# casinca/LLM-quest

Measured on AMD Instinct MI355X. Metric: img+tokens/sec fwd+bwd, ViT-B+Qwen3-0.6B VLM, 224px+512tok, higher is better.
Workload: dtype bf16; 1 GPU; BASELINE configs[3]: VLM early fusion, ViT-B/16 (frozen, fwd) + ffn adapter 768->3072->1024 + Qwen3-0.6B, 224x224 image + 512 text tokens (S=709), fwd+loss+bwd, no optimizer step; per_gpu_batch=160, global_batch=160, parallelism=dp1, text_mask=all ones, vision_tower_precision=bf16 MFMA operands, fp32 residual stream

## Files before the change

### llm_quest_amd/csrc/attention.hip

```cpp
#include "attn_common.h"

namespace {

template <int D>
__global__ __launch_bounds__(256, 2) void attn_fwd_kernel(int B, int S, int Hq, int Hkv, const bf16_t* __restrict__ q, int64_t ldq,
                                                          const bf16_t* __restrict__ k, int64_t ldk, const bf16_t* __restrict__ v,
                                                          int64_t ldv, bf16_t* __restrict__ o, int64_t ldo, float* __restrict__ lse,
                                                          const uint8_t* __restrict__ key_mask, int causal, float scale_log2) {
    using C = Cfg<D>;
    const int abl = causal >> 8;
    causal &= 0xff;
    __shared__ __attribute__((aligned(16))) char smem[4 * C::TILE];
    const int lane = threadIdx.x & 63;
    const int wave = __builtin_amdgcn_readfirstlane(threadIdx.x >> 6);
    const int nqb = (S + 127) / 128;
    const int vid = (abl >> 8) & 1 ? (int)blockIdx.x : xcd_chunked((int)blockIdx.x, (int)gridDim.x);
    const int qb = nqb - 1 - (vid % nqb);
    const int bh = vid / nqb;
    const int hq = bh % Hq, b = bh / Hq;
    const int hkv = hq / (Hq / Hkv);
    const int q0 = qb * 128;
    const int qg = q0 + wave * 32 + (lane & 31);
    const bool qvalid = qg < S;

// ... 282 lines not shown

    for (int kt = 0; kt < ntiles; ++kt) {
        [[maybe_unused]] const unsigned long long t_sync = PROF_T();
        wait_vmcnt<0>();
        __syncthreads();
        PROF_ADD(1, t_sync);
        const int nv = S - kt * 64;
        unsigned long long kbits = nv >= 64 ? ~0ull : ((1ull << nv) - 1ull);
        if (mrow) kbits &= __ballot(mk != 0);
        [[maybe_unused]] const unsigned long long t_iss = PROF_T();
        const bool more = kt + 1 < ntiles;
        const bool spread = more && S - (kt + 1) * 64 >= 64 && !(abl & 512);
        if (more && !spread) issue(kt + 1, (kt + 1) & 1);
        const auto nkr = __builtin_amdgcn_make_buffer_rsrc(const_cast<bf16_t*>(kbase + (int64_t)(kt + 1) * 64 * ldk), 0, 0x7fffffff, 0x00020000);
        const auto nvr = __builtin_amdgcn_make_buffer_rsrc(const_cast<bf16_t*>(vbase + (int64_t)(kt + 1) * 64 * ldv), 0, 0x7fffffff, 0x00020000);
        char* const nst = smem + ((kt + 1) & 1) * 2 * C::TILE;
        auto piece = [&](auto i_) {
            constexpr int i = i_.value;
            if constexpr (i < C::PPW) {
                const int row = (wave * C::PPW + i) * C::RPP + prow;
                __builtin_amdgcn_raw_ptr_buffer_load_lds(nkr, LDS_PTR(nst + (wave * C::PPW + i) * 1024), 16, dk_row + (unsigned)(swz_row<D>(pch, row) << 4), (int)(i * C::RPP * ldk * 2), 0, 0);
            } else {
                constexpr int j = i - C::PPW;
                const int row = (wave * C::PPW + j) * C::RPP + prow;
                __builtin_amdgcn_raw_ptr_buffer_load_lds(nvr, LDS_PTR(nst + C::TILE + (wave * C::PPW + j) * 1024), 16, dv_row + (unsigned)(swz_tr<D>(pch, row) << 4), (int)(j * C::RPP * ldv * 2), 0, 0);
            }
        };
        PROF_ADD(2, t_iss);
        if (mrow) mk = mrow[min((kt + 1) * 64 + lane, S - 1)];
        [[maybe_unused]] unsigned long long t_seg = PROF_T();
        if (prof_on) prof_acc[7] += 1;
        const int koff = (kt & 1) * 2 * C::TILE, voff = koff + C::TILE;
        if (causal && !allt && kt * 64 > qw + 31) continue;
        int vkx[C::KS], vv[C::DT];
#pragma unroll
        for (int ks = 0; ks < C::KS; ++ks) vkx[ks] = (lo.row + koff) ^ (ks << 5);
#pragma unroll
        for (int dt = 0; dt < C::DT; ++dt) vv[dt] = lo.col[dt] + voff;
        f32x16 sacc[2];
        static_assert(2 * C::PPW == C::KS, "one next-tile piece behind every second MFMA of the S product");
        auto s_product = [&](auto spread_c) {
            static_for<2>([&](auto st_) {
                constexpr int st = st_.value;
                static_for<C::KS>([&](auto ks_) {
                    constexpr int ks = ks_.value, m = st * C::KS + ks;
                    sacc[st] = __builtin_amdgcn_mfma_f32_32x32x16_bf16(lds_frag(smem, vkx[ks], st * 32 * C::ROWB), qf[ks], ks == 0 ? ninit : sacc[st], 0, 0, 0);
                    if constexpr (decltype(spread_c)::value && m % 2 == 1) piece(std::integral_constant<int, m / 2>{});
                });
            });
        };
        if (spread) s_product(std::true_type{});
        else s_product(std::false_type{});
        TrHalves ft[2][C::DT];
        auto issue_v = [&](auto g_) {
            constexpr int g = g_.value, imm = 16 * g * C::ROWB;
            static_for<C::DT>([&](auto dt_) { tr_issue<imm, imm + 8 * C::ROWB>(ft[g & 1][dt_.value], lds0 + vv[dt_.value], lds0 + vv[dt_.value]); });
        };
        issue_v(std::integral_constant<int, 0>{});
#if ATTN_ABL & 16
        asm volatile("" : "+v"(sacc[0]), "+v"(sacc[1]));
        if (prof_on) { const unsigned long long now = __builtin_readcyclecounter(); prof_acc[3] += now - t_seg; t_seg = now; }
#endif
        if ((kbits != ~0ull) || allt || (causal && kt * 64 + 63 > qw)) {
            const unsigned long long exist = nv >= 64 ? ~0ull : ((1ull << nv) - 1ull);
            unsigned m16[2], x16[2];
#pragma unroll
            for (int st = 0; st < 2; ++st) {
                const unsigned sh = 4u * (unsigned)(lane >> 5);
                const unsigned vis = lean_gather16((st ? (unsigned)(kbits >> 32) : (unsigned)kbits) >> sh);
                x16[st] = lean_gather16((st ? (unsigned)(exist >> 32) : (unsigned)exist) >> sh);
                const int x = qw - kt * 64 - st * 32;
                const unsigned cz = (!causal || x >= 32) ? 0u : (x == 0 ? tri16 : 0xFFFFu);
                m16[st] = (~vis & 0xFFFFu) | cz;
            }
            const unsigned mall = m16[0] | (m16[1] << 16), eall = x16[0] | (x16[1] << 16);
            const unsigned mset = qrow ? ~eall : mall;
#pragma unroll
            for (int st = 0; st < 2; ++st)
#pragma unroll
                for (int ee = 0; ee < 16; ++ee) sacc[st][ee] = lean_set_if(sacc[st][ee], mset, 16 * st + ee, LEAN_FILL);
            if (allt) {
                const unsigned zset = qrow ? eall : 0u;
#pragma unroll
                for (int st = 0; st < 2; ++st)
#pragma unroll
                    for (int ee = 0; ee < 16; ++ee) sacc[st][ee] = lean_set_if(sacc[st][ee], zset, 16 * st + ee, 0u);
            }
        }
        float t0 = lean_max3(sacc[0][0], sacc[0][1], sacc[0][2]), t1 = lean_max3(sacc[1][0], sacc[1][1], sacc[1][2]);
#pragma unroll
        for (int e = 3; e < 15; e += 2) {
            t0 = lean_max3(t0, sacc[0][e], sacc[0][e + 1]);
            t1 = lean_max3(t1, sacc[1][e], sacc[1][e + 1]);
        }
        float t = lean_max3(t0, t1, sacc[0][15]);
        t = lean_max3(t, sacc[1][15], __shfl_xor(lean_max3(t, sacc[1][15], sacc[1][15]), 32, 64));
// ... 43 lines not shown
                oacc[dt] = __builtin_amdgcn_mfma_f32_32x32x16_bf16(tr_wait<younger>(ft[g & 1][dt]), pf, oacc[dt], 0, 0, 0);
            });
        });
#if ATTN_ABL & 16
        asm volatile("" : "+v"(oacc[0]), "+v"(oacc[1]));
        PROF_ADD(5, t_seg);
        if (prof_on) prof_acc[6] += 1;
#endif
    }
#if ATTN_ABL & 16
    PROF_ADD(0, t_wg);
    if (prof_on && (abl & 4096) && (blockIdx.x & 63) == 5)
        for (int i = 0; i < 16; ++i) atomicAdd(&g_prof[i], prof_acc[i]);
#endif

    l += __shfl_xor(l, 32, 64);
    const float inv = 1.0f / l;
    if (abl & 32) {
        bf16_t* orow = o + ((int64_t)b * S + qg) * ldo + (int64_t)hq * D + 8 * (lane >> 5);
#pragma unroll
        for (int dt = 0; dt < C::DT; ++dt)
#pragma unroll
            for (int gp = 0; gp < 2; ++gp) {
                const int r0 = 8 * gp;
                const unsigned a0 = pack_bf2(oacc[dt][r0] * inv, oacc[dt][r0 + 1] * inv), a1 = pack_bf2(oacc[dt][r0 + 2] * inv, oacc[dt][r0 + 3] * inv);
                const unsigned b0 = pack_bf2(oacc[dt][r0 + 4] * inv, oacc[dt][r0 + 5] * inv), b1 = pack_bf2(oacc[dt][r0 + 6] * inv, oacc[dt][r0 + 7] * inv);
                const auto s0 = __builtin_amdgcn_permlane32_swap(a0, b0, false, false), s1 = __builtin_amdgcn_permlane32_swap(a1, b1, false, false);
                const u32x4 w = {s0[0], s1[0], s0[1], s1[1]};
                if (qvalid) *reinterpret_cast<u32x4*>(orow + dt * 32 + 16 * gp) = w;
            }
    } else {
        constexpr int RB = 2 * D, PCS = RB / 16;
        __syncthreads();
        {
            const int row = wave * 32 + (lane & 31), hb = lane >> 5;
#pragma unroll
            for (int dt = 0; dt < C::DT; ++dt)
#pragma unroll
                for (int g4 = 0; g4 < 4; ++g4) {
                    const int chunk = dt * 8 + 2 * g4 + hb;
                    const u32x2 pk = {pack_bf2(oacc[dt][4 * g4] * inv, oacc[dt][4 * g4 + 1] * inv), pack_bf2(oacc[dt][4 * g4 + 2] * inv, oacc[dt][4 * g4 + 3] * inv)};
                    *reinterpret_cast<u32x2*>(smem + row * RB + (((chunk >> 1) ^ (row & (PCS - 1))) << 4) + (chunk & 1) * 8) = pk;
                }
        }
        __syncthreads();
#pragma unroll
        for (int it = 0; it < 128 * PCS / 256; ++it) {
            const int i = it * 256 + (int)threadIdx.x, row = i / PCS, pc = i % PCS;
            const u32x4 w = *reinterpret_cast<const u32x4*>(smem + row * RB + ((pc ^ (row & (PCS - 1))) << 4));
            if (q0 + row < S) *reinterpret_cast<u32x4*>(o + ((int64_t)b * S + q0 + row) * ldo + (int64_t)hq * D + pc * 8) = w;
        }
    }
    if (qvalid && lane < 32) lse[((int64_t)b * Hq + hq) * S + qg] = ((qrow ? MASK_T : mref) + __builtin_amdgcn_logf(l)) * LN2;
}

template <int D>
__global__ __launch_bounds__(256) void attn_delta_kernel(int B, int S, int Hq, const bf16_t* __restrict__ o, int64_t ldo,
                                                         const bf16_t* __restrict__ d_o, int64_t lddo, float* __restrict__ delta,
                                                         const float* __restrict__ lse, float* __restrict__ nl2, float* __restrict__ ndl) {
    constexpr int LPR = D / 8, RPW = 64 / LPR;
    const int lane = threadIdx.x & 63, sub = lane / LPR, li = lane % LPR;
    const int hgroups = (Hq + RPW - 1) / RPW;
    const int64_t total = (int64_t)B * S * hgroups;
    for (int64_t item = (int64_t)blockIdx.x * 4 + (threadIdx.x >> 6); item < total; item += (int64_t)gridDim.x * 4) {
        const int64_t tok = item / hgroups;
        const int h = (int)(item - tok * hgroups) * RPW + sub;
        float s = 0.f;
// ... 161 lines not shown
                    } else if constexpr (!(ATTN_ABL & 4)) {
                        constexpr int h = g - 2 * NA, st = h / NC, sd = (h % NC) / DT, dt = h % DT;
                        const u32x4 w = {dsw[st][4 * sd], dsw[st][4 * sd + 1], dsw[st][4 * sd + 2], dsw[st][4 * sd + 3]};
                        constexpr int younger = NG - 1 - g < PD ? NG - 1 - g : PD;
                        mfma_owned<OWNED, 16 * dt>(tr_wait<2 * younger>(ft[g % RING]), __builtin_bit_cast(bf16x8, w));
                    }
                    if constexpr (g == NA) tiles_settle(sacc[0], pacc[0]);
                    if constexpr (g == 2 * NA) tiles_settle(sacc[1], pacc[1]);
                    if constexpr (g >= NA && g < 2 * NA) {
                        constexpr int m = g - NA, per = 16 / NA;
                        static_for<per>([&](auto i) { element(std::integral_constant<int, 0>{}, std::integral_constant<int, m * per + i.value>{}); });
                    } else if constexpr (g >= 2 * NA && g < 2 * NA + NC) {
                        constexpr int m = g - 2 * NA, per = 16 / NC;
                        static_for<per>([&](auto i) { element(std::integral_constant<int, 1>{}, std::integral_constant<int, m * per + i.value>{}); });
                    }
                    __builtin_amdgcn_sched_barrier(0);
                });
            };
            if (boundary) tile_body(std::true_type{});
            else tile_body(std::false_type{});
        }
        owned_settle<OWNED>();
        bf16_t* row = dq + ((int64_t)b * S + qg) * lddq + (int64_t)hq * D;
        static_for<DT * 4>([&](auto i) {
            constexpr int dt = i.value / 4, g4 = i.value % 4, r = 16 * dt + 4 * g4;
            const int d = dt * 32 + 8 * g4 + 4 * (lane >> 5);
            const u32x2 pk = {pack_bf2(owned_read<OWNED, r>() * scale, owned_read<OWNED, r + 1>() * scale),
                              pack_bf2(owned_read<OWNED, r + 2>() * scale, owned_read<OWNED, r + 3>() * scale)};
            if (qvalid && !(abl & 2)) *reinterpret_cast<u32x2*>(row + d) = pk;
        });
    }
}

template <int D, bool LEAN>
__global__ __launch_bounds__(256, 1) void attn_bwd_dkv_kernel(int B, int S, int Hq, int Hkv, const bf16_t* __restrict__ q, int64_t ldq,
                                                              const bf16_t* __restrict__ k, int64_t ldk, const bf16_t* __restrict__ v,
                                                              int64_t ldv, const bf16_t* __restrict__ d_o, int64_t lddo,
                                                              const float* __restrict__ lse, const float* __restrict__ delta,
                                                              bf16_t* __restrict__ dk, int64_t lddk, bf16_t* __restrict__ dv, int64_t lddv,
                                                              const uint8_t* __restrict__ key_mask, int causal, float scale, float scale_log2,
                                                              int bpw, bf16_t* __restrict__ ds_out) {
    using C = Cfg<D>;
    constexpr int KS = C::KS, DT = C::DT;
    constexpr int NA = 2 * KS, NC = 4 * DT, NG = 2 * NA + 2 * NC;
    constexpr int OWNED = 32 * DT + 8 * KS, DK0 = 16 * DT, KF0 = 32 * DT, VF0 = KF0 + 4 * KS;
    constexpr int RING = ATTN_RING, PD = ATTN_PD;
    constexpr bool UNI = C::UNI;
    constexpr int NIMG = UNI ? 2 : 4, NST = 3, STAGE = NIMG * C::TILE, PIECES = NIMG * C::PPW;
    constexpr int OIMG = (UNI ? 1 : 2) * C::TILE;
    const int abl = causal >> 8;
    causal &= 0xff;
    __shared__ __attribute__((aligned(16))) char smem[NST * STAGE + NST * 512];
    char* rowc = smem + NST * STAGE;
    const int lane = threadIdx.x & 63;
    const int wave = __builtin_amdgcn_readfirstlane(threadIdx.x >> 6);
    const int nkb = (S + 127) / 128, nchunk = (nkb + bpw - 1) / bpw;
    const int chunk = blockIdx.x % nchunk, bh = blockIdx.x / nchunk;
    const int hkv = bh % Hkv, b = bh / Hkv;
    const int rep = Hq / Hkv;
    const int kb_lo = chunk * bpw, kb_hi = min(nkb, kb_lo + bpw);
    const int nqt_all = (S + 63) / 64;
    auto qt0_of = [&](int kb) { return causal ? kb * 2 : 0; };

    int ikb = kb_lo, ih = 0, iq = 0, istage = 0;
    auto issue_next = [&]() -> bool {
        if (ikb < kb_hi && iq >= nqt_all - qt0_of(ikb)) { iq = 0; ++ih; }
// ... 38 lines not shown
    auto request_kv = [&](int kb_) {
        const int kg_ = kb_ * 128 + wave * 32 + (lane & 31);
        load_rows_frag<D>(k + (int64_t)b * S * ldk + (int64_t)hkv * D, ldk, kg_, kg_ < S, lane, tk);
        load_rows_frag<D>(v + (int64_t)b * S * ldv + (int64_t)hkv * D, ldv, kg_, kg_ < S, lane, tv);
    };
    if (kb_lo < kb_hi) request_kv(kb_lo);
    for (int kb = kb_lo; kb < kb_hi; ++kb) {
        [[maybe_unused]] const unsigned long long t_pro = PROF_T();
        const int k0 = kb * 128;
        const int kg = k0 + wave * 32 + (lane & 31);
        const bool kvalid = kg < S;
        const bool kreal = kvalid && (key_mask == nullptr || key_mask[(int64_t)b * S + kg] != 0);
        owned_zero<OWNED, 0, 32 * DT>();
        if constexpr (LEAN) {
#pragma unroll
            for (int ks = 0; ks < KS; ++ks) {
                u32x4 w = __builtin_bit_cast(u32x4, tk[ks]);
#pragma unroll
                for (int e = 0; e < 4; ++e) w[e] = pack_bf2(__uint_as_float(w[e] << 16) * scale_log2, __uint_as_float(w[e] & 0xffff0000u) * scale_log2);
                tk[ks] = __builtin_bit_cast(bf16x8, w);
            }
        }
        static_for<KS>([&](auto ks) { owned_write4<OWNED, KF0 + 4 * ks.value>(tk[ks.value]); });
        static_for<KS>([&](auto ks) { owned_write4<OWNED, VF0 + 4 * ks.value>(tv[ks.value]); });
        const int qt0 = qt0_of(kb);
        const int per_head = nqt_all - qt0;
        const int nit = per_head * rep;
        PROF_ADD(3, t_pro);
        int ch = 0, cq = -1;
        for (int it = 0; it < nit; ++it) {
            if (++cq == per_head) { cq = 0; ++ch; }
            [[maybe_unused]] const unsigned long long t_w = PROF_T();
            if (inflight >= 2) {
                if (st1 + st2 == 8) wait_vmcnt<PIECES + 1 + 8>();
                else if (st1 + st2 == 4) wait_vmcnt<PIECES + 1 + 4>();
                else wait_vmcnt<PIECES + 1>();
            } else wait_vmcnt<0>();
            st2 = st1;
            st1 = 0;
            PROF_ADD(1, t_w);
            [[maybe_unused]] const unsigned long long t_b = PROF_T();
            __builtin_amdgcn_s_barrier();
            PROF_ADD(6, t_b);
            --inflight;
            [[maybe_unused]] const unsigned long long t_i = PROF_T();
            if (!(abl & 1)) inflight += issue_next();
            PROF_ADD(7, t_i);
#if ATTN_ABL & 16
            struct BodyTimer {
                unsigned long long t0; bool on; unsigned long long* acc;
                __device__ ~BodyTimer() { if (on) { acc[2] += __builtin_readcyclecounter() - t0; acc[5] += 1; } }
            } body_timer{PROF_T(), prof_on, prof_acc};
#endif
            const int qt = qt0 + cq;
            const int qroff = cstage * STAGE, qtoff = UNI ? qroff : qroff + C::TILE, oroff = qroff + OIMG, otoff = UNI ? oroff : oroff + C::TILE;
            const float* rc = reinterpret_cast<const float*>(rowc + cstage * 512) + 4 * (lane >> 5);
            cstage = cstage == NST - 1 ? 0 : cstage + 1;
            if (causal && qt * 64 + 63 < k0 + wave * 32) continue;
            const bool boundary = (causal && qt * 64 < k0 + wave * 32 + 31) || (qt * 64 + 64 > S) || __any(!kreal);
            int vqx[KS], vox[KS], vqt[DT], vot[DT];
#pragma unroll
            for (int ks = 0; ks < KS; ++ks) {
                vqx[ks] = ((UNI ? lo.rowu : lo.row) + qroff) ^ (ks << 5);
                vox[ks] = ((UNI ? lo.rowu : lo.row) + oroff) ^ (ks << 5);
            }
#pragma unroll
            for (int dt = 0; dt < DT; ++dt) {
                vqt[dt] = (UNI ? lo.colu[dt] : lo.col[dt]) + qtoff;
                vot[dt] = (UNI ? lo.colu[dt] : lo.col[dt]) + otoff;
            }

            auto tile_body = [&](auto bc) {
                constexpr bool BOUNDARY = decltype(bc)::value;
                bf16x8 f[RING] = {};
                TrHalves ft[RING] = {};
                f32x16 sacc[2], pacc[2];
                unsigned pw[2][8] = {}, dsw[2][8] = {};
                float lsr[2][16], dlr[2][16], tt[2][16], pv[2][16], dsv[2][16];
                [[maybe_unused]] f32x16 linit[2], dinit[2];
                auto load = [&](auto gc) {
                    constexpr int g = gc.value;
                    if constexpr (ATTN_ABL & 1) return;
                    if constexpr (g < 2 * NA) {
                        constexpr int st = g / NA, ks = (g % NA) / 2, which = g % 2;
                        f[g % RING] = lds_frag(smem, which ? vox[ks] : vqx[ks], st * 32 * C::ROWB);
                    } else if constexpr (g < NG) {
                        constexpr int h = g - 2 * NA, st = h / NC, sd = (h % NC) / (2 * DT), dt = (h % (2 * DT)) / 2, which = h % 2;
                        constexpr int imm = (st * 32 + 16 * sd) * C::ROWB;
                        const int va = which ? vqt[dt] : vot[dt];
                        if constexpr (!(ATTN_ABL & 32)) tr_issue<imm, imm + 8 * C::ROWB>(ft[g % RING], lds0 + va, lds0 + (UNI ? va ^ 0x20 : va));
                    }
                };
                auto row_constants = [&](auto stc) {
                    constexpr int st = stc.value;
#pragma unroll
                    for (int g4 = 0; g4 < 4; ++g4) {
                        const f32x4 a = *reinterpret_cast<const f32x4*>(rc + st * 32 + 8 * g4);
                        const f32x4 c = *reinterpret_cast<const f32x4*>(rc + 64 + st * 32 + 8 * g4);
#pragma unroll
                        for (int e = 0; e < 4; ++e) {
                            if constexpr (LEAN) {
                                linit[st][4 * g4 + e] = a[e];
                                dinit[st][4 * g4 + e] = c[e];
                            } else {
                                lsr[st][4 * g4 + e] = a[e];
                                dlr[st][4 * g4 + e] = c[e];
                            }
                        }
                    }
                };
                auto stage = [&](auto stc, auto ec, auto kc) {
                    constexpr int st = stc.value, e = ec.value, k = kc.value;
                    if constexpr (e < 0 || e >= 16 || (ATTN_ABL & 2)) return;
                    else if constexpr (LEAN) {
                        if constexpr (k == 1 && BOUNDARY) {
                            const int qq = qt * 64 + st * 32 + acc_row(e, lane);
                            const bool masked = (causal && kg > qq) || !kreal || qq >= S;
                            sacc[st][e] = masked ? -INFINITY : sacc[st][e];
                            asm volatile("" : "+v"(sacc[st][e]));
                        } else if constexpr (k == 2) {
                            pv[st][e] = __builtin_amdgcn_exp2f(sacc[st][e]);
                            asm volatile("" : "+v"(pv[st][e]));
                        } else if constexpr (k == 3) {
                            dsv[st][e] = pacc[st][e] * pv[st][e];
                            if constexpr (e % 2 == 1) {
                                pw[st][e / 2] = pack_bf2(pv[st][e - 1], pv[st][e]);
                                dsw[st][e / 2] = pack_bf2(dsv[st][e - 1], dsv[st][e]);
                                asm volatile("" : "+v"(pw[st][e / 2]), "+v"(dsw[st][e / 2]));
                            } else {
                                asm volatile("" : "+v"(dsv[st][e]));
                            }
                        }
                    } else if constexpr (k == 0) {
                        lsr[st][e] *= LOG2E;
                        asm volatile("" : "+v"(lsr[st][e]));
                    } else if constexpr (k == 1) {
                        float t = fmaf(sacc[st][e], scale_log2, -lsr[st][e]);
                        if constexpr (BOUNDARY) {
                            const int qq = qt * 64 + st * 32 + acc_row(e, lane);
                            const bool masked = (causal && kg > qq) || !kreal || qq >= S;
                            t = masked ? -INFINITY : t;
                        }
                        tt[st][e] = t;
                        asm volatile("" : "+v"(tt[st][e]));
                    } else if constexpr (k == 2) {
                        pv[st][e] = __builtin_amdgcn_exp2f(tt[st][e]);
                        dsv[st][e] = pacc[st][e] - dlr[st][e];
                        asm volatile("" : "+v"(pv[st][e]), "+v"(dsv[st][e]));
                    } else {
                        dsv[st][e] *= pv[st][e];
                        if constexpr (e % 2 == 1) {
                            pw[st][e / 2] = pack_bf2(pv[st][e - 1], pv[st][e]);
                            dsw[st][e / 2] = pack_bf2(dsv[st][e - 1], dsv[st][e]);
                            asm volatile("" : "+v"(pw[st][e / 2]), "+v"(dsw[st][e / 2]));
                        } else {
                            asm volatile("" : "+v"(dsv[st][e]));
                        }
                    }
                };
                auto b_step = [&](auto stc, auto mc, auto perc) {
                    constexpr int m = mc.value, PER = perc.value;
                    if constexpr (m >= 0 && m < 16 / PER + 3)
                        static_for<4>([&](auto kc) {
                            static_for<PER>([&](auto i) { stage(stc, std::integral_constant<int, (m - kc.value) * PER + i.value>{}, kc); });
                        });
                };
                if constexpr (LEAN) row_constants(std::integral_constant<int, 0>{});
                static_for<PD>([&](auto g) { load(g); });
                [[maybe_unused]] unsigned long long t_seg = PROF_T();
                static_for<NG>([&](auto gc) {
                    constexpr int g = gc.value;
#if ATTN_ABL & 16
                    if constexpr (g == NA || g == 2 * NA || g == 2 * NA + NC) {
                        if (prof_on) { const unsigned long long now = __builtin_readcyclecounter(); prof_acc[8 + (g == NA ? 0 : g == 2 * NA ? 1 : 2)] += now - t_seg; t_seg = now; }
                    }
#endif
                    if constexpr (!LEAN && g == NA - 1) row_constants(std::integral_constant<int, 0>{});
                    if constexpr (LEAN && g == NA - 4) row_constants(std::integral_constant<int, 1>{});
                    load(std::integral_constant<int, g + PD>{});
                    if constexpr (g < 2 * NA) {
                        constexpr int st = g / NA, ks = (g % NA) / 2, which = g % 2;
                        if constexpr ((ATTN_ABL & 8) && ks > 0) {
                        } else if constexpr (LEAN && ks == 0) {
                            if constexpr (which == 0) mfma_ownedB_init<OWNED, KF0>(sacc[st], f[g % RING], linit[st]);
                            else mfma_ownedB_init<OWNED, VF0>(pacc[st], f[g % RING], dinit[st]);
                        } else if constexpr (which == 0) mfma_ownedB<OWNED, KF0 + 4 * ks, ks == 0>(sacc[st], f[g % RING]);
                        else mfma_ownedB<OWNED, VF0 + 4 * ks, ks == 0>(pacc[st], f[g % RING]);
                    } else if constexpr (!(ATTN_ABL & 4)) {
                        constexpr int h = g - 2 * NA, st = h / NC, sd = (h % NC) / (2 * DT), dt = (h % (2 * DT)) / 2, which = h % 2;
                        constexpr int younger = NG - 1 - g < PD ? NG - 1 - g : PD;
                        const bf16x8 fa = tr_wait<2 * younger>(ft[g % RING]);
                        if constexpr (which == 0) {
                            const u32x4 w = {pw[st][4 * sd], pw[st][4 * sd + 1], pw[st][4 * sd + 2], pw[st][4 * sd + 3]};
                            mfma_owned<OWNED, 16 * dt, false>(fa, __builtin_bit_cast(bf16x8, w));
                        } else {
                            const u32x4 w = {dsw[st][4 * sd], dsw[st][4 * sd + 1], dsw[st][4 * sd + 2], dsw[st][4 * sd + 3]};
                            mfma_owned<OWNED, DK0 + 16 * dt, false>(fa, __builtin_bit_cast(bf16x8, w));
                        }
                    }
                    if constexpr (g == NA) tiles_settle(sacc[0], pacc[0]);
                    if constexpr (g == 2 * NA) tiles_settle(sacc[1], pacc[1]);
                    static_assert(16 % NA == 0 && 16 % NC == 0 && 16 / (16 / NA) + 3 <= NA + NC / 2 && 16 / (16 / NC) + 3 <= NC + NC / 2, "B phase does not fit its gaps");
                    b_step(std::integral_constant<int, 0>{}, std::integral_constant<int, g - NA>{}, std::integral_constant<int, 16 / NA>{});
                    b_step(std::integral_constant<int, 1>{}, std::integral_constant<int, g - 2 * NA>{}, std::integral_constant<int, 16 / NC>{});
                    if constexpr (!LEAN && g == 2 * NA - 1) row_constants(std::integral_constant<int, 1>{});
                    __builtin_amdgcn_sched_barrier(0);
                });
                PROF_ADD(11, t_seg);
                if (ds_out) {
                    const int hq_ = hkv * rep + ch;
                    const int nqb_ = (S + 127) / 128;
                    char* blk = reinterpret_cast<char*>(ds_out) + ((((int64_t)b * Hq + hq_) * (2 * nqb_) + qt) * 2 * (4 * nqb_) + (kb * 4 + wave)) * 2048 + lane * 16;
                    static_for<4>([&](auto i) {
                        constexpr int st = i.value / 2, c2 = i.value % 2;
                        const u32x4 w4 = {dsw[st][4 * c2], dsw[st][4 * c2 + 1], dsw[st][4 * c2 + 2], dsw[st][4 * c2 + 3]};
                        *reinterpret_cast<u32x4*>(blk + (int64_t)st * (4 * nqb_) * 2048 + c2 * 1024) = w4;
                    });
                }
            };
            if (boundary) tile_body(std::true_type{});
            else tile_body(std::false_type{});
            st1 = ds_out != nullptr ? 4 : 0;
        }
        [[maybe_unused]] const unsigned long long t_epi = PROF_T();
        owned_settle<OWNED>();
        if (kb + 1 < kb_hi) request_kv(kb + 1);
        bf16_t* krow = dk + ((int64_t)b * S + kg) * lddk + (int64_t)hkv * D + 8 * (lane >> 5);
        bf16_t* vrow = dv + ((int64_t)b * S + kg) * lddv + (int64_t)hkv * D + 8 * (lane >> 5);
        static_for<DT * 2>([&](auto i) {
            constexpr int dt = i.value / 2, gp = i.value % 2, rv = 16 * dt + 8 * gp, rk = DK0 + rv;
            const unsigned ka0 = pack_bf2(owned_read<OWNED, rk>() * scale, owned_read<OWNED, rk + 1>() * scale), ka1 = pack_bf2(owned_read<OWNED, rk + 2>() * scale, owned_read<OWNED, rk + 3>() * scale);
            const unsigned kb0 = pack_bf2(owned_read<OWNED, rk + 4>() * scale, owned_read<OWNED, rk + 5>() * scale), kb1 = pack_bf2(owned_read<OWNED, rk + 6>() * scale, owned_read<OWNED, rk + 7>() * scale);
            const unsigned va0 = pack_bf2(owned_read<OWNED, rv>(), owned_read<OWNED, rv + 1>()), va1 = pack_bf2(owned_read<OWNED, rv + 2>(), owned_read<OWNED, rv + 3>());
            const unsigned vb0 = pack_bf2(owned_read<OWNED, rv + 4>(), owned_read<OWNED, rv + 5>()), vb1 = pack_bf2(owned_read<OWNED, rv + 6>(), owned_read<OWNED, rv + 7>());
            const auto k0s = __builtin_amdgcn_permlane32_swap(ka0, kb0, false, false), k1s = __builtin_amdgcn_permlane32_swap(ka1, kb1, false, false);
            const auto v0s = __builtin_amdgcn_permlane32_swap(va0, vb0, false, false), v1s = __builtin_amdgcn_permlane32_swap(va1, vb1, false, false);
            const u32x4 wk = {k0s[0], k1s[0], k0s[1], k1s[1]}, wv = {v0s[0], v1s[0], v0s[1], v1s[1]};
            if (kvalid && !(abl & 2)) {
                *reinterpret_cast<u32x4*>(krow + dt * 32 + 16 * gp) = wk;
                *reinterpret_cast<u32x4*>(vrow + dt * 32 + 16 * gp) = wv;
            }
        });
        PROF_ADD(4, t_epi);
    }
    PROF_ADD(0, t_wg);
#if ATTN_ABL & 16
    if (prof_on)
        for (int i = 0; i < 16; ++i) atomicAdd(&g_prof[i], prof_acc[i]);
#endif
}

struct QkFuse {
    const bf16_t* qkv;
    int64_t ldqkv;
    const bf16_t* qw;
// ... 21 lines not shown
#if DQ_ABL & 16
__device__ unsigned long long g_dq_prof[32];
#define DQ_T() __builtin_readcyclecounter()
#define DQ_MARK(i) do { const unsigned long long now_ = __builtin_readcyclecounter(); dqp[i] += now_ - dq_t; dq_t = now_; } while (0)
#else
#define DQ_T() 0ull
#define DQ_MARK(i) do { } while (0)
#endif
template <int D, bool FUSE>
__global__ __launch_bounds__(256, 2) void attn_bwd_dq_spill_kernel(int B, int S, int Hq, int Hkv, const bf16_t* __restrict__ k, int64_t ldk,
                                                                   const bf16_t* __restrict__ ds, bf16_t* __restrict__ dq, int64_t lddq,
                                                                   int causal, float scale, QkFuse f) {
    using C = Cfg<D>;
    constexpr int DT = C::DT, DSW = 4096;
    constexpr int KST = 2, DST = 3, DS_BASE = KST * C::TILE, DS_STAGE = 4 * DSW;
    __shared__ __attribute__((aligned(16))) char smem[KST * C::TILE + DST * DS_STAGE];
    const int lane = threadIdx.x & 63;
    const int wave = __builtin_amdgcn_readfirstlane(threadIdx.x >> 6);
    const int nqb = (S + 127) / 128;
    const int vid = xcd_chunked((int)blockIdx.x, (int)gridDim.x);
    int qb, bh;
    heavy_first(vid, nqb, B * Hq, ATTN_HEAD_GROUP, qb, bh);
    const int hq = bh % Hq, b = bh / Hq;
    const int hkv = hq / (Hq / Hkv);
    const int q0 = qb * 128;
    const int qw = q0 + wave * 32;
    const int qg = qw + (lane & 31);
    const int ntiles_all = (S + 63) / 64;
    const int ntiles = causal ? min(ntiles_all, (q0 + 127) / 64 + 1) : ntiles_all;
    const bf16_t* kbase = k + (int64_t)b * S * ldk + (int64_t)hkv * D;
    const char* sblk = reinterpret_cast<const char*>(ds) + (((((int64_t)b * Hq + hq) * (2 * nqb) + 2 * qb + (wave >> 1)) * 2 + (wave & 1)) * (4 * nqb)) * 2048;
    auto srsrc = __builtin_amdgcn_make_buffer_rsrc(const_cast<char*>(sblk), 0, 0x7fffffff, 0x00020000);
    const unsigned unit = (unsigned)(lane ^ ((lane >> 5) << 2)) * 16;
    auto fetched = [&](int kgrp) { return !(causal && kgrp * 32 > qw + 31) && kgrp * 32 < S; };
    auto issue_k = [&](int kt) {
        if (!((DQ_ABL & 2) && kt > 0)) dma_tile<D, IMG_TR>(kbase + (int64_t)kt * 64 * ldk, ldk, S - kt * 64, smem + (kt % KST) * C::TILE, wave, lane);
    };
    auto issue_ds = [&](int kt) {
        char* mine = smem + DS_BASE + (kt % DST) * DS_STAGE + wave * DSW;
#pragma unroll
        for (int half = 0; half < 2; ++half) {
            const bool live = fetched(2 * kt + half) && kt < ntiles && !((DQ_ABL & 1) && kt > 0);
            const unsigned o0 = live ? (unsigned)((2 * kt + half) * 2048) + unit : OOB;
            const unsigned o1 = live ? (unsigned)((2 * kt + half) * 2048 + 1024) + unit : OOB;
            __builtin_amdgcn_raw_ptr_buffer_load_lds(srsrc, LDS_PTR(mine + half * 2048), 16, o0, 0, 0, 0);
            __builtin_amdgcn_raw_ptr_buffer_load_lds(srsrc, LDS_PTR(mine + half * 2048 + 1024), 16, o1, 0, 0, 0);
        }
    };
    const LaneOff<D> lok = lane_offsets<D>(lane);
    const int g = lane >> 4, q4 = (lane >> 2) & 3, p = lane & 3;
    const unsigned scol = (unsigned)((g & 1) * 1024 + ((((p & 1) * 32 + 4 * (g >> 1) + q4) ^ ((p & 1) << 2)) * 16) + (p >> 1) * 8) + DS_BASE + wave * DSW;
    const unsigned lds0 = (unsigned)(unsigned long long)LDS_PTR(smem);
    f32x16 acc[DT];
#pragma unroll
    for (int i = 0; i < DT; ++i)
#pragma unroll
        for (int e = 0; e < 16; ++e) acc[i][e] = 0.f;
    [[maybe_unused]] unsigned long long dqp[8] = {};
    [[maybe_unused]] unsigned long long dq_t = DQ_T();
    [[maybe_unused]] const unsigned long long dq_t0 = dq_t;
    [[maybe_unused]] int pos_pre[4] = {0, 0, 0, 0};
    if constexpr (FUSE) {
#pragma unroll
        for (int it = 0; it < 4; ++it) {
            const int qrow = q0 + (int)(threadIdx.x >> 3) + 32 * it;
            pos_pre[it] = f.pos[(int64_t)b * S + (qrow < S ? qrow : S - 1)];
        }
// ... 493 lines not shown
```

### llm_quest_amd/csrc/attn_common.h

```cpp
#pragma once
#include <type_traits>

#include "common.h"

namespace {

constexpr float MASK_T = -2.0e38f;
constexpr float LOG2E = 1.4426950408889634f;
constexpr float LN2 = 0.6931471805599453f;
constexpr unsigned OOB = 0x80000000u;
constexpr int ATTN_MAX_TILES = 512;

template <int D>
struct Cfg {
    static constexpr int ROWB = D * 2;
    static constexpr int CH = ROWB / 16;
    static constexpr int KS = D / 16;
    static constexpr int DT = D / 32;
    static constexpr int TILE = 64 * ROWB;
    static constexpr int RPP = 1024 / ROWB;
    static constexpr int PPW = TILE / 1024 / 4;
    static constexpr bool UNI = (D == 128);
};

// ... 189 lines not shown
    static_assert(OFF % 4 == 0 && OFF + 4 <= OWNED, "operand outside the owned range");
    constexpr int R0 = 256 - OWNED + OFF;
    if constexpr (FIRST) OWNED_ASM(OWNED, "v_mfma_f32_32x32x16_bf16 %0, %1, a[%c2:%c3], 0" : "=&v"(acc) : "v"(a), "i"(R0), "i"(R0 + 3));
    else OWNED_ASM(OWNED, "v_mfma_f32_32x32x16_bf16 %0, %1, a[%c2:%c3], %0" : "+v"(acc) : "v"(a), "i"(R0), "i"(R0 + 3));
}
template <int OWNED, int OFF>
__device__ __forceinline__ void mfma_ownedB_init(f32x16& acc, const bf16x8& a, const f32x16& init) {
    static_assert(OFF % 4 == 0 && OFF + 4 <= OWNED, "operand outside the owned range");
    constexpr int R0 = 256 - OWNED + OFF;
    OWNED_ASM(OWNED, "v_mfma_f32_32x32x16_bf16 %0, %1, a[%c3:%c4], %2" : "=&v"(acc) : "v"(a), "v"(init), "i"(R0), "i"(R0 + 3));
}
__device__ __forceinline__ void tiles_settle(f32x16& x, f32x16& y) { asm volatile("s_nop 15\n\ts_nop 3" : "+v"(x), "+v"(y)); }
template <int OWNED, int OFF, int COUNT>
__device__ __forceinline__ void owned_zero() {
    static_for<COUNT>([&](auto r) { OWNED_ASM(OWNED, "v_accvgpr_write_b32 a[%c0], 0" ::"i"(256 - OWNED + OFF + r.value)); });
}
template <int OWNED, int OFF>
__device__ __forceinline__ void owned_write4(const bf16x8& v) {
    const u32x4 w = __builtin_bit_cast(u32x4, v);
    OWNED_ASM(OWNED, "v_accvgpr_write_b32 a[%c4], %0\n\tv_accvgpr_write_b32 a[%c5], %1\n\tv_accvgpr_write_b32 a[%c6], %2\n\tv_accvgpr_write_b32 a[%c7], %3"
              ::"v"(w[0]), "v"(w[1]), "v"(w[2]), "v"(w[3]), "i"(256 - OWNED + OFF), "i"(256 - OWNED + OFF + 1), "i"(256 - OWNED + OFF + 2), "i"(256 - OWNED + OFF + 3));
}
template <int OWNED>
__device__ __forceinline__ void owned_settle() { OWNED_ASM(OWNED, "s_nop 15\n\ts_nop 3" ::); }
template <int OWNED, int R>
__device__ __forceinline__ float owned_read() {
    float x;
    asm volatile("v_accvgpr_read_b32 %0, a[%c1]" : "=v"(x) : "i"(256 - OWNED + R));
    return x;
}

__device__ __forceinline__ int acc_row(int e, int lane) { return (e & 3) + 8 * (e >> 2) + 4 * (lane >> 5); }

__device__ __forceinline__ int xcd_chunked(int b, int n) {
    const int xcd = b & 7, q = n >> 3, r = n & 7;
    return (xcd < r ? xcd * (q + 1) : r * (q + 1) + (xcd - r) * q) + (b >> 3);
}

}
```

### llm_quest_amd/fingerprint.py

```python

import hashlib
import json
import os
import re

_HERE = os.path.dirname(os.path.abspath(__file__))
EVIDENCE_ROUND = "r06"
FILES = ("attention.hip", "attn_common.h", "elementwise.hip", "gemm.hip", "norm_rope.hip", "common.h")
_FLAG_LINES = re.compile(r"^(CXXFLAGS|ARCH|FLAGS_(?:attention|elementwise|gemm|norm_rope))\s*\??=")


def compile_flags():
    out = []
    with open(os.path.join(_HERE, "csrc", "Makefile")) as fh:
        for line in fh:
            if _FLAG_LINES.match(line):
                out.append(" ".join(line.split()))
    return "\n".join(out)


def kernel_sources_sha():
    h = hashlib.sha256()
    for n in FILES:
        h.update(n.encode())
        with open(os.path.join(_HERE, "csrc", n), "rb") as fh:
            h.update(fh.read())
    h.update(compile_flags().encode())
    return h.hexdigest()[:16]


def all_sources_sha():
    h = hashlib.sha256()
    d = os.path.join(_HERE, "csrc")
    for n in sorted(f for f in os.listdir(d) if f.endswith((".hip", ".h")) and not f.startswith("_")):
        h.update(n.encode())
        with open(os.path.join(d, n), "rb") as fh:
            h.update(fh.read())
    with open(os.path.join(d, "Makefile")) as fh:
        h.update("\n".join(" ".join(line.split()) for line in fh if re.match(r"^(CXXFLAGS|ARCH|FLAGS_\w+)\s*\??=", line)).encode())
    return h.hexdigest()[:16]
# ... 18 lines not shown
```

Before: 190,100 img+tok/s.

## Specialize attention boundary tiles by mask mode and skip dead query rows

Adds compile-time mask modes (diagonal, ragged rows, fully masked, dead half) to the lean backward dK/dV tile body. Boundary tiles no longer take the generic per-element masking path, and a half-trip schedule drops the MFMAs for query subtiles past the sequence end. The forward kernel gains a cheap constant-lane diagonal mask and skips work for waves whose query rows are all beyond S, and the dQ kernel stops fetching for such rows. The cost is more template instantiations, a more complex wait-count ladder, and a risk of masking or scheduling mistakes in the specialized paths.

Measured after the change: 191,100 img+tok/s, median of 6. About the same (+0.5%).

```diff
diff --git a/llm_quest_amd/csrc/attention.hip b/llm_quest_amd/csrc/attention.hip
--- a/llm_quest_amd/csrc/attention.hip
+++ b/llm_quest_amd/csrc/attention.hip
@@ -338,6 +338,10 @@
         if (prof_on) prof_acc[7] += 1;
         const int koff = (kt & 1) * 2 * C::TILE, voff = koff + C::TILE;
         if (causal && !allt && kt * 64 > qw + 31) continue;
+        if (qw >= S) {
+            if (spread) static_for<2 * C::PPW>(piece);
+            continue;
+        }
         int vkx[C::KS], vv[C::DT];
 #pragma unroll
         for (int ks = 0; ks < C::KS; ++ks) vkx[ks] = (lo.row + koff) ^ (ks << 5);
@@ -367,7 +371,20 @@
         asm volatile("" : "+v"(sacc[0]), "+v"(sacc[1]));
         if (prof_on) { const unsigned long long now = __builtin_readcyclecounter(); prof_acc[3] += now - t_seg; t_seg = now; }
 #endif
-        if ((kbits != ~0ull) || allt || (causal && kt * 64 + 63 > qw)) {
+        if (D == 128 && kbits == ~0ull && !allt) {
+            if (causal && kt * 64 + 63 > qw) {
+                static_for<2>([&](auto st_) {
+                    constexpr int st = st_.value;
+                    const int x = qw - kt * 64 - st * 32;
+                    if (x == 0) {
+                        static_for<16>([&](auto ee) { sacc[st][ee.value] = keep_lanes_c<diag_visible<true>(ee.value)>(sacc[st][ee.value], MASK_T); });
+                    } else if (x < 0) {
+#pragma unroll
+                        for (int ee = 0; ee < 16; ++ee) sacc[st][ee] = MASK_T;
+                    }
+                });
+            }
+        } else if ((kbits != ~0ull) || allt || (causal && kt * 64 + 63 > qw)) {
             const unsigned long long exist = nv >= 64 ? ~0ull : ((1ull << nv) - 1ull);
             unsigned m16[2], x16[2];
 #pragma unroll
@@ -477,7 +494,7 @@
     } else {
         constexpr int RB = 2 * D, PCS = RB / 16;
         __syncthreads();
-        {
+        if (qw < S) {
             const int row = wave * 32 + (lane & 31), hb = lane >> 5;
 #pragma unroll
             for (int dt = 0; dt < C::DT; ++dt)
@@ -705,6 +722,7 @@
     }
 }
 
+constexpr int M_NONE = 0, M_DIAG = 1, M_ROWS = 2, M_FULL = 3, M_GEN = 4, M_DEAD = 5;
 template <int D, bool LEAN>
 __global__ __launch_bounds__(256, 1) void attn_bwd_dkv_kernel(int B, int S, int Hq, int Hkv, const bf16_t* __restrict__ q, int64_t ldq,
                                                               const bf16_t* __restrict__ k, int64_t ldk, const bf16_t* __restrict__ v,
@@ -809,8 +827,11 @@
             if (++cq == per_head) { cq = 0; ++ch; }
             [[maybe_unused]] const unsigned long long t_w = PROF_T();
             if (inflight >= 2) {
-                if (st1 + st2 == 8) wait_vmcnt<PIECES + 1 + 8>();
-                else if (st1 + st2 == 4) wait_vmcnt<PIECES + 1 + 4>();
+                const int sts = st1 + st2;
+                if (sts >= 8) wait_vmcnt<PIECES + 1 + 8>();
+                else if (sts >= 6) wait_vmcnt<PIECES + 1 + 6>();
+                else if (sts >= 4) wait_vmcnt<PIECES + 1 + 4>();
+                else if (sts >= 2) wait_vmcnt<PIECES + 1 + 2>();
                 else wait_vmcnt<PIECES + 1>();
             } else wait_vmcnt<0>();
             st2 = st1;
@@ -847,25 +868,52 @@
                 vot[dt] = (UNI ? lo.colu[dt] : lo.col[dt]) + otoff;
             }
 
-            auto tile_body = [&](auto bc) {
-                constexpr bool BOUNDARY = decltype(bc)::value;
+            auto tile_body = [&](auto m0c, auto m1c) {
+                constexpr int M0 = decltype(m0c)::value, M1 = decltype(m1c)::value;
+                constexpr bool HALF = M1 == M_DEAD;
+                constexpr int NGR = HALF ? NA + NC : NG;
+                static_assert(!HALF || (LEAN && NA == 16 && NC == 16), "the half trip is scheduled for head_dim 128, lean form");
+                static_assert(LEAN || ((M0 == M_NONE || M0 == M_GEN) && M0 == M1), "the recompute form keeps its two bodies");
                 bf16x8 f[RING] = {};
                 TrHalves ft[RING] = {};
                 f32x16 sacc[2], pacc[2];
                 unsigned pw[2][8] = {}, dsw[2][8] = {};
                 float lsr[2][16], dlr[2][16], tt[2][16], pv[2][16], dsv[2][16];
                 [[maybe_unused]] f32x16 linit[2], dinit[2];
-                auto load = [&](auto gc) {
-                    constexpr int g = gc.value;
+                auto load = [&](auto ic) {
+                    constexpr int i = ic.value, g = HALF && i >= NA ? i + NA : i;
                     if constexpr (ATTN_ABL & 1) return;
-                    if constexpr (g < 2 * NA) {
+                    if constexpr (i >= NGR) return;
+                    else if constexpr (g < 2 * NA) {
                         constexpr int st = g / NA, ks = (g % NA) / 2, which = g % 2;
-                        f[g % RING] = lds_frag(smem, which ? vox[ks] : vqx[ks], st * 32 * C::ROWB);
-                    } else if constexpr (g < NG) {
+                        f[i % RING] = lds_frag(smem, which ? vox[ks] : vqx[ks], st * 32 * C::ROWB);
+                    } else {
                         constexpr int h = g - 2 * NA, st = h / NC, sd = (h % NC) / (2 * DT), dt = (h % (2 * DT)) / 2, which = h % 2;
                         constexpr int imm = (st * 32 + 16 * sd) * C::ROWB;
                         const int va = which ? vqt[dt] : vot[dt];
-                        if constexpr (!(ATTN_ABL & 32)) tr_issue<imm, imm + 8 * C::ROWB>(ft[g % RING], lds0 + va, lds0 + (UNI ? va ^ 0x20 : va));
+                        if constexpr (!(ATTN_ABL & 32)) tr_issue<imm, imm + 8 * C::ROWB>(ft[i % RING], lds0 + va, lds0 + (UNI ? va ^ 0x20 : va));
+                    }
+                };
+                auto masked_score = [&](auto stc, auto ec, float x) -> float {
+                    constexpr int st = stc.value, e = ec.value, MODE = st ? M1 : M0;
+                    if constexpr (MODE == M_GEN) {
+                        const int qq = qt * 64 + st * 32 + acc_row(e, lane);
+                        const bool masked = (causal && kg > qq) || !kreal || qq >= S;
+                        return masked ? -INFINITY : x;
+                    } else {
+                        return x;
+                    }
+                };
+                auto masked_p = [&](auto stc, auto ec, float p) -> float {
+                    constexpr int st = stc.value, e = ec.value, MODE = st ? M1 : M0;
+                    if constexpr (MODE == M_DIAG) {
+                        return keep_lanes_or_zero_c<diag_visible<false>(e)>(p);
+                    } else {
+                        static_assert(MODE == M_ROWS, "a lane-set mode");
+                        constexpr int r = (e & 3) + 8 * (e >> 2);
+                        const int n = S - qt * 64 - st * 32;
+                        const unsigned long long vis = (r < n ? 0xffffffffull : 0ull) | (r + 4 < n ? 0xffffffff00000000ull : 0ull);
+                        return keep_lanes_or_zero(p, vis);
                     }
                 };
                 auto row_constants = [&](auto stc) {
@@ -890,11 +938,19 @@
                     constexpr int st = stc.value, e = ec.value, k = kc.value;
                     if constexpr (e < 0 || e >= 16 || (ATTN_ABL & 2)) return;
                     else if constexpr (LEAN) {
-                        if constexpr (k == 1 && BOUNDARY) {
-                            const int qq = qt * 64 + st * 32 + acc_row(e, lane);
-                            const bool masked = (causal && kg > qq) || !kreal || qq >= S;
-                            sacc[st][e] = masked ? -INFINITY : sacc[st][e];
+                        constexpr int MODE = st ? M1 : M0;
+                        if constexpr (k == 1 && MODE == M_GEN) {
+                            sacc[st][e] = masked_score(stc, ec, sacc[st][e]);
                             asm volatile("" : "+v"(sacc[st][e]));
+                        } else if constexpr (k == 1 && (MODE == M_DIAG || MODE == M_ROWS)) {
+                            pv[st][e] = __builtin_amdgcn_exp2f(sacc[st][e]);
+                            asm volatile("" : "+v"(pv[st][e]));
+                        } else if constexpr (k == 2 && (MODE == M_DIAG || MODE == M_ROWS)) {
+                            pv[st][e] = masked_p(stc, ec, pv[st][e]);
+                            asm volatile("" : "+v"(pv[st][e]));
+                        } else if constexpr (k == 2 && MODE == M_FULL) {
+                            pv[st][e] = 0.f;
+                            asm volatile("" : "+v"(pv[st][e]));
                         } else if constexpr (k == 2) {
                             pv[st][e] = __builtin_amdgcn_exp2f(sacc[st][e]);
                             asm volatile("" : "+v"(pv[st][e]));
@@ -913,11 +969,7 @@
                         asm volatile("" : "+v"(lsr[st][e]));
                     } else if constexpr (k == 1) {
                         float t = fmaf(sacc[st][e], scale_log2, -lsr[st][e]);
-                        if constexpr (BOUNDARY) {
-                            const int qq = qt * 64 + st * 32 + acc_row(e, lane);
-                            const bool masked = (causal && kg > qq) || !kreal || qq >= S;
-                            t = masked ? -INFINITY : t;
-                        }
+                        t = masked_score(stc, ec, t);
                         tt[st][e] = t;
                         asm volatile("" : "+v"(tt[st][e]));
                     } else if constexpr (k == 2) {
@@ -945,42 +997,54 @@
                 if constexpr (LEAN) row_constants(std::integral_constant<int, 0>{});
                 static_for<PD>([&](auto g) { load(g); });
                 [[maybe_unused]] unsigned long long t_seg = PROF_T();
-                static_for<NG>([&](auto gc) {
-                    constexpr int g = gc.value;
+                static_for<NGR>([&](auto ic) {
+                    constexpr int i = ic.value, g = HALF && i >= NA ? i + NA : i;
 #if ATTN_ABL & 16
                     if constexpr (g == NA || g == 2 * NA || g == 2 * NA + NC) {
                         if (prof_on) { const unsigned long long now = __builtin_readcyclecounter(); prof_acc[8 + (g == NA ? 0 : g == 2 * NA ? 1 : 2)] += now - t_seg; t_seg = now; }
                     }
 #endif
                     if constexpr (!LEAN && g == NA - 1) row_constants(std::integral_constant<int, 0>{});
-                    if constexpr (LEAN && g == NA - 4) row_constants(std::integral_constant<int, 1>{});
-                    load(std::integral_constant<int, g + PD>{});
+                    if constexpr (LEAN && !HALF && g == NA - 4) row_constants(std::integral_constant<int, 1>{});
+                    load(std::integral_constant<int, i + PD>{});
                     if constexpr (g < 2 * NA) {
                         constexpr int st = g / NA, ks = (g % NA) / 2, which = g % 2;
                         if constexpr ((ATTN_ABL & 8) && ks > 0) {
                         } else if constexpr (LEAN && ks == 0) {
-                            if constexpr (which == 0) mfma_ownedB_init<OWNED, KF0>(sacc[st], f[g % RING], linit[st]);
-                            else mfma_ownedB_init<OWNED, VF0>(pacc[st], f[g % RING], dinit[st]);
-                        } else if constexpr (which == 0) mfma_ownedB<OWNED, KF0 + 4 * ks, ks == 0>(sacc[st], f[g % RING]);
-                        else mfma_ownedB<OWNED, VF0 + 4 * ks, ks == 0>(pacc[st], f[g % RING]);
+                            if constexpr (which == 0) mfma_ownedB_init<OWNED, KF0>(sacc[st], f[i % RING], linit[st]);
+                            else mfma_ownedB_init<OWNED, VF0>(pacc[st], f[i % RING], dinit[st]);
+                        } else if constexpr (which == 0) mfma_ownedB<OWNED, KF0 + 4 * ks, ks == 0>(sacc[st], f[i % RING]);
+                        else mfma_ownedB<OWNED, VF0 + 4 * ks, ks == 0>(pacc[st], f[i % RING]);
                     } else if constexpr (!(ATTN_ABL & 4)) {
                         constexpr int h = g - 2 * NA, st = h / NC, sd = (h % NC) / (2 * DT), dt = (h % (2 * DT)) / 2, which = h % 2;
-                        constexpr int younger = NG - 1 - g < PD ? NG - 1 - g : PD;
-                        const bf16x8 fa = tr_wait<2 * younger>(ft[g % RING]);
+                        constexpr int younger = NGR - 1 - i < PD ? NGR - 1 - i : PD;
+                        const bf16x8 fa = tr_wait<2 * younger>(ft[i % RING]);
                         if constexpr (which == 0) {
                             const u32x4 w = {pw[st][4 * sd], pw[st][4 * sd + 1], pw[st][4 * sd + 2], pw[st][4 * sd + 3]};
-                            mfma_owned<OWNED, 16 * dt, false>(fa, __builtin_bit_cast(bf16x8, w));
+                            mfma_owned<OWNED, 16 * dt, HALF>(fa, __builtin_bit_cast(bf16x8, w));
                         } else {
                             const u32x4 w = {dsw[st][4 * sd], dsw[st][4 * sd + 1], dsw[st][4 * sd + 2], dsw[st][4 * sd + 3]};
-                            mfma_owned<OWNED, DK0 + 16 * dt, false>(fa, __builtin_bit_cast(bf16x8, w));
+                            mfma_owned<OWNED, DK0 + 16 * dt, HALF>(fa, __builtin_bit_cast(bf16x8, w));
                         }
                     }
-                    if constexpr (g == NA) tiles_settle(sacc[0], pacc[0]);
-                    if constexpr (g == 2 * NA) tiles_settle(sacc[1], pacc[1]);
                     static_assert(16 % NA == 0 && 16 % NC == 0 && 16 / (16 / NA) + 3 <= NA + NC / 2 && 16 / (16 / NC) + 3 <= NC + NC / 2, "B phase does not fit its gaps");
-                    b_step(std::integral_constant<int, 0>{}, std::integral_constant<int, g - NA>{}, std::integral_constant<int, 16 / NA>{});
-                    b_step(std::integral_constant<int, 1>{}, std::integral_constant<int, g - 2 * NA>{}, std::integral_constant<int, 16 / NC>{});
-                    if constexpr (!LEAN && g == 2 * NA - 1) row_constants(std::integral_constant<int, 1>{});
+                    if constexpr (!HALF) {
+                        if constexpr (g == NA) tiles_settle(sacc[0], pacc[0]);
+                        if constexpr (g == 2 * NA) tiles_settle(sacc[1], pacc[1]);
+                        b_step(std::integral_constant<int, 0>{}, std::integral_constant<int, g - NA>{}, std::integral_constant<int, 16 / NA>{});
+                        b_step(std::integral_constant<int, 1>{}, std::integral_constant<int, g - 2 * NA>{}, std::integral_constant<int, 16 / NC>{});
+                    } else {
+                        constexpr int BARE = 8 + 3;
+                        if constexpr (g == NA - 1) {
+                            tiles_settle(sacc[0], pacc[0]);
+                            static_for<BARE>([&](auto mc) {
+                                b_step(std::integral_constant<int, 0>{}, mc, std::integral_constant<int, 1>{});
+                                __builtin_amdgcn_sched_barrier(0);
+                            });
+                        }
+                        if constexpr (g >= 2 * NA) b_step(std::integral_constant<int, 0>{}, std::integral_constant<int, BARE + g - 2 * NA>{}, std::integral_constant<int, 1>{});
+                    }
+                    if constexpr (!LEAN && !HALF && g == 2 * NA - 1) row_constants(std::integral_constant<int, 1>{});
                     __builtin_amdgcn_sched_barrier(0);
                 });
                 PROF_ADD(11, t_seg);
@@ -988,16 +1052,35 @@
                     const int hq_ = hkv * rep + ch;
                     const int nqb_ = (S + 127) / 128;
                     char* blk = reinterpret_cast<char*>(ds_out) + ((((int64_t)b * Hq + hq_) * (2 * nqb_) + qt) * 2 * (4 * nqb_) + (kb * 4 + wave)) * 2048 + lane * 16;
-                    static_for<4>([&](auto i) {
+                    static_for<(HALF ? 2 : 4)>([&](auto i) {
                         constexpr int st = i.value / 2, c2 = i.value % 2;
                         const u32x4 w4 = {dsw[st][4 * c2], dsw[st][4 * c2 + 1], dsw[st][4 * c2 + 2], dsw[st][4 * c2 + 3]};
                         *reinterpret_cast<u32x4*>(blk + (int64_t)st * (4 * nqb_) * 2048 + c2 * 1024) = w4;
                     });
                 }
             };
-            if (boundary) tile_body(std::true_type{});
-            else tile_body(std::false_type{});
-            st1 = ds_out != nullptr ? 4 : 0;
+            using std::integral_constant;
+            if constexpr (!LEAN) {
+                if (boundary) tile_body(integral_constant<int, M_GEN>{}, integral_constant<int, M_GEN>{});
+                else tile_body(integral_constant<int, M_NONE>{}, integral_constant<int, M_NONE>{});
+                st1 = ds_out != nullptr ? 4 : 0;
+            } else {
+                int md[2];
+#pragma unroll
+                for (int st = 0; st < 2; ++st) {
+                    const int x = qt * 64 + 32 * st - (k0 + wave * 32), n = S - qt * 64 - 32 * st;
+                    const bool diag = causal && x == 0;
+                    md[st] = n <= 0 ? M_DEAD : (causal && x < 0) ? M_FULL : (diag && n < 32) ? M_GEN : diag ? M_DIAG : n < 32 ? M_ROWS : M_NONE;
+                }
+                const bool plain = !__any(!kreal);
+                st1 = ds_out != nullptr ? (md[1] == M_DEAD ? 2 : 4) : 0;
+                if (!boundary) tile_body(integral_constant<int, M_NONE>{}, integral_constant<int, M_NONE>{});
+                else if (plain && md[0] == M_DIAG && md[1] == M_NONE) tile_body(integral_constant<int, M_DIAG>{}, integral_constant<int, M_NONE>{});
+                else if (plain && md[0] == M_FULL && md[1] == M_DIAG) tile_body(integral_constant<int, M_FULL>{}, integral_constant<int, M_DIAG>{});
+                else if (plain && md[0] == M_ROWS && md[1] == M_DEAD) tile_body(integral_constant<int, M_ROWS>{}, integral_constant<int, M_DEAD>{});
+                else if (md[1] == M_DEAD) tile_body(integral_constant<int, M_GEN>{}, integral_constant<int, M_DEAD>{});
+                else tile_body(integral_constant<int, M_GEN>{}, integral_constant<int, M_GEN>{});
+            }
         }
         [[maybe_unused]] const unsigned long long t_epi = PROF_T();
         owned_settle<OWNED>();
@@ -1085,7 +1168,7 @@
     const char* sblk = reinterpret_cast<const char*>(ds) + (((((int64_t)b * Hq + hq) * (2 * nqb) + 2 * qb + (wave >> 1)) * 2 + (wave & 1)) * (4 * nqb)) * 2048;
     auto srsrc = __builtin_amdgcn_make_buffer_rsrc(const_cast<char*>(sblk), 0, 0x7fffffff, 0x00020000);
     const unsigned unit = (unsigned)(lane ^ ((lane >> 5) << 2)) * 16;
-    auto fetched = [&](int kgrp) { return !(causal && kgrp * 32 > qw + 31) && kgrp * 32 < S; };
+    auto fetched = [&](int kgrp) { return !(causal && kgrp * 32 > qw + 31) && kgrp * 32 < S && qw < S; };
     auto issue_k = [&](int kt) {
         if (!((DQ_ABL & 2) && kt > 0)) dma_tile<D, IMG_TR>(kbase + (int64_t)kt * 64 * ldk, ldk, S - kt * 64, smem + (kt % KST) * C::TILE, wave, lane);
     };
diff --git a/llm_quest_amd/csrc/attn_common.h b/llm_quest_amd/csrc/attn_common.h
--- a/llm_quest_amd/csrc/attn_common.h
+++ b/llm_quest_amd/csrc/attn_common.h
@@ -245,6 +245,36 @@
 
 __device__ __forceinline__ int acc_row(int e, int lane) { return (e & 3) + 8 * (e >> 2) + 4 * (lane >> 5); }
 
+template <unsigned long long VIS>
+__device__ __forceinline__ float keep_lanes_c(float x, float fill) {
+    float r;
+    asm("s_mov_b32 vcc_lo, %c3\n\ts_mov_b32 vcc_hi, %c4\n\tv_cndmask_b32 %0, %2, %1, vcc"
+        : "=v"(r) : "v"(x), "v"(fill), "n"((unsigned)(VIS & 0xffffffffull)), "n"((unsigned)(VIS >> 32)) : "vcc");
+    return r;
+}
+template <unsigned long long VIS>
+__device__ __forceinline__ float keep_lanes_or_zero_c(float x) {
+    float r;
+    asm("s_mov_b32 vcc_lo, %c2\n\ts_mov_b32 vcc_hi, %c3\n\tv_cndmask_b32 %0, 0, %1, vcc"
+        : "=v"(r) : "v"(x), "n"((unsigned)(VIS & 0xffffffffull)), "n"((unsigned)(VIS >> 32)) : "vcc");
+    return r;
+}
+__device__ __forceinline__ float keep_lanes_or_zero(float x, unsigned long long vis) {
+    float r;
+    asm("s_mov_b64 vcc, %2\n\tv_cndmask_b32 %0, 0, %1, vcc" : "=v"(r) : "v"(x), "s"(vis) : "vcc");
+    return r;
+}
+template <bool ROWS_ARE_KEYS>
+constexpr unsigned long long diag_visible(int e) {
+    const int r = (e & 3) + 8 * (e >> 2);
+    unsigned long long m = 0;
+    for (int lane = 0; lane < 64; ++lane) {
+        const int row = r + 4 * (lane >> 5), col = lane & 31;
+        if (ROWS_ARE_KEYS ? row <= col : col <= row) m |= 1ull << lane;
+    }
+    return m;
+}
+
 __device__ __forceinline__ int xcd_chunked(int b, int n) {
     const int xcd = b & 7, q = n >> 3, r = n & 7;
     return (xcd < r ? xcd * (q + 1) : r * (q + 1) + (xcd - r) * q) + (b >> 3);
diff --git a/llm_quest_amd/fingerprint.py b/llm_quest_amd/fingerprint.py
--- a/llm_quest_amd/fingerprint.py
+++ b/llm_quest_amd/fingerprint.py
@@ -5,7 +5,7 @@
 import re
 
 _HERE = os.path.dirname(os.path.abspath(__file__))
-EVIDENCE_ROUND = "r06"
+EVIDENCE_ROUND = "r07"
 FILES = ("attention.hip", "attn_common.h", "elementwise.hip", "gemm.hip", "norm_rope.hip", "common.h")
 _FLAG_LINES = re.compile(r"^(CXXFLAGS|ARCH|FLAGS_(?:attention|elementwise|gemm|norm_rope))\s*\??=")
 
```
